# deepsound-project/pggan-pytorch

Hardware: AMD Instinct MI355X
Metric: images/sec, PGGAN full train step (D+GP step + G step + Adam) at 1024x1024 (higher is better)
Workload: dtype f32; 1 GPU; BASELINE config 5: PGGAN 1024x1024 net (fmap_base 4096, C=3, latent 512), stage depth 8 = 1024x1024, alpha 1.00, minibatch 3/GPU (reference schedule), Trainer.train(): WGAN-GP + Adam(0,0.99) at lr 0, fp32; resolution=1024, depth=8, minibatch_per_gpu=3, global_batch=3, parallelism=dp1, fmap_base=4096, hip_graphs=False

## Files before the change

### include/pggan_hip_debug.h

```cpp
#ifndef PGGAN_HIP_DEBUG_H
#define PGGAN_HIP_DEBUG_H

#ifdef __cplusplus
extern "C" {
#endif

const char* pg_debug_last_conv_kernel(void);
const char* pg_debug_last_wino_kernel(void);
const char* pg_debug_last_wino_wgrad_kernel(void);

enum pg_tune_key {
    PG_TUNE_CONV_TILE = 0,
    PG_TUNE_WGRAD = 1,
    PG_TUNE_SPLITK = 2,
    PG_TUNE_PATH = 3
};
enum pg_wgrad_cfg {
    PG_WGRAD_32x16_128PX = 1,
    PG_WGRAD_64x16_64PX = 3,
    PG_WGRAD_TILE_NOT_STRIP = 20
};
enum pg_path {
    PG_PATH_NO_THIN = 2,
    PG_PATH_NO_SMALLMAP_SPLIT = 8,
    PG_PATH_SMALLMAP_SPLIT_2304 = 9,
    PG_PATH_UNFUSED_PIXELNORM = 11,
    PG_PATH_NO_THIN_POOL16 = 17,
    PG_PATH_TILE_NOT_STRIP = 20,
    PG_PATH_K4_ONE_WORKGROUP = 21
};
int pg_debug_set_tuning(int key, int value);
int pg_debug_set_wino(int vec);
int pg_debug_set_wino_ksplit(int n);
int pg_debug_set_wino_epi(int mode);

#ifdef __cplusplus
}
#endif
#endif
```

### pggan-pytorch_amd/csrc/conv_api.hip

```cpp
#include "convp.h"

__thread char pgk::g_last_kernel[96] = "";
__thread int pgk::g_tune[4] = {-1, -1, -1, -1};

namespace {

using namespace pgk;

__device__ __forceinline__ void pack_dgrad_tile(const float* __restrict__ w, float* __restrict__ wt, int KS, int Cout, int Cin,
                                                int tap, int ci_b, int co_b)
{
    __shared__ float tile[32][33];
    const int kh = tap / KS, kw = tap % KS;
    const int otap = (KS - 1 - kh) * KS + (KS - 1 - kw);
    const int tx = threadIdx.x & 31, ty = threadIdx.x >> 5;
    for (int r = ty; r < 32; r += 8) {
        const int co = co_b + r, ci = ci_b + tx;
        tile[r][tx] = (co < Cout && ci < Cin) ? w[((size_t)tap * Cout + co) * Cin + ci] : 0.f;
    }
    __syncthreads();
    for (int r = ty; r < 32; r += 8) {
        const int ci = ci_b + r, co = co_b + tx;
        if (ci < Cin && co < Cout) wt[((size_t)otap * Cin + ci) * Cout + co] = tile[tx][r];
    }
// ... 32 lines not shown
    if (want.ypool && !pooled)
        return pg_avgpool2_fwd(want.y, want.pool_other, want.ypool, want.N, want.Hout >> 1, want.Wout >> 1, want.Cout, want.pool_a, want.pool_b, stream);
    if (want.yup) return pg_avgpool2_bwd(want.y, want.upmask, want.yup, want.N, want.Hout, want.Wout, want.Cout, want.up_mul, want.mask_slope, stream);
    if (want.pn_r) return pg_pixelnorm_fwd(want.y, want.y, want.pn_r, P, want.Cout, want.pn_eps, stream);
    if (want.pnb_y) return pg_pixelnorm_lrelu_bwd(want.y, want.pnb_y, want.pnb_r, want.y, P, want.Cout, want.mask_slope, stream);
    return 0;
}

static bool thin_shape(const ConvP& p, bool channels)
{
    return channels && p.KS == 3 && p.pad == 1 && (p.Wout & 31) == 0 && (p.Hout & 7) == 0 && g_tune[PG_TUNE_PATH] != PG_PATH_NO_THIN;
}

static ConvP conv_request(const float* x, const float* w, const float* bias, const float* mask, float* y,
                          int N, int Hin, int Win, int Cin, int Cout, int KS, int pad, float scale, float slope, float mask_slope)
{
    ConvP p;
    p.x = x; p.w = w; p.bias = bias; p.mask = mask; p.y = y;
    p.N = N; p.Hin = Hin; p.Win = Win; p.Cin = Cin; p.Cout = Cout; p.KS = KS; p.pad = pad;
    p.scale = scale; p.slope = slope; p.mask_slope = mask_slope;
    return p;
}

static int conv2d_impl(ConvP& p, int flags, pg_stream_t stream)
{
    if (!p.x || !p.w || !p.y || p.N <= 0 || p.Hin <= 0 || p.Win <= 0 || p.Cin <= 0 || p.Cout <= 0) return PG_E_ARG;
    if ((p.Cin & 3) || (p.Cout & 3)) return PG_E_ALIGN;
    const int KS = p.KS, Cin = p.Cin, Cout = p.Cout;
    p.ups = flags & PG_FLAG_UPSAMPLE;
    p.mask_bytes = (flags & PG_FLAG_MASK_BYTES) ? 1 : 0; p.y_bytes = (flags & PG_FLAG_Y_BYTES) ? 1 : 0;
    if (flags & PG_FLAG_SIGNS_OUT) {
        if (!p.mask || p.mask_bytes) return PG_E_ARG;
        p.ysigns = reinterpret_cast<unsigned char*>(const_cast<float*>(p.mask));
        p.mask = nullptr;
    }
    p.Hout = p.Hin + 2 * p.pad - KS + 1; p.Wout = p.Win + 2 * p.pad - KS + 1;
    if (p.Hout <= 0 || p.Wout <= 0 || !is_pow2(p.Hout) || !is_pow2(p.Wout)) return PG_E_UNSUP;
    if (p.ups && ((p.Hin | p.Win) & 1)) return PG_E_ARG;
    if (p.ypool && ((p.Hout | p.Wout) & 1)) return PG_E_ARG;
    if ((long long)p.N * p.Hin * p.Win * Cin >= (1ll << 31) || (long long)p.N * p.Hout * p.Wout * Cout >= (1ll << 31) ||
        (long long)KS * KS * Cout * Cin >= (1ll << 31)) return PG_E_UNSUP;
    const ConvP want = p;
    if (KS != 3) p.ypool = nullptr;
    p.yup = nullptr; p.pn_r = nullptr; p.pnb_y = nullptr;
    hipStream_t s = (hipStream_t)stream;
    int rc;
    if (p.mask_bytes || p.y_bytes || p.ysigns) {
        if (KS != 3 || (p.y_bytes && !p.ypool) || want.pn_r || want.pnb_y) return PG_E_UNSUP;
        p.yup = want.yup;
        const bool thin_plain = !p.y_bytes && !p.yup && !p.ypool && ((Cout == 8 && (Cin == 8 || Cin == 16)) || (Cout == 16 && Cin == 8 && p.mask));
        const bool thin_pool = g_tune[PG_TUNE_PATH] != PG_PATH_NO_THIN_POOL16 && !p.yup && p.ypool && Cout == 16 && Cin == 8;
        return thin_shape(p, thin_plain || thin_pool) ? dispatch_thin(p, s) : dispatch_conv_tile(p, s);
    }
    const bool thin_pn = thin_shape(p, Cout == 8 && (Cin == 8 || Cin == 16));
    if (want.pnb_y && want.pnb_r && KS == 3 && Cout <= 32) {
        p.pnb_y = want.pnb_y;
        rc = thin_pn ? dispatch_thin(p, s) : dispatch_conv_tile(p, s);
        if (rc != PG_E_UNSUP) return rc;
        p.pnb_y = nullptr;
    }
    if (want.pn_r && KS == 3 && Cout <= 32 && !p.mask && g_tune[PG_TUNE_PATH] != PG_PATH_UNFUSED_PIXELNORM) {
        p.pn_r = want.pn_r;
        rc = thin_pn ? dispatch_thin(p, s) : dispatch_conv_tile(p, s);
        if (rc != PG_E_UNSUP) return rc;
// ... 10 lines not shown
    else if (k4_layer(p, KS))
        rc = launch_k4_conv(p, s);
    else
        rc = dispatch_conv_tile(p, s);
    if (rc) return rc;
    return second_pass(want, p.ypool && p.ksplit == 1, stream);
}

extern "C" int pg_conv2d_nhwc(const float* x, const float* w, const float* bias, const float* mask, float* y,
                              int N, int Hin, int Win, int Cin, int Cout, int KS, int pad, int ups,
                              float scale, float slope, float mask_slope, pg_stream_t stream)
{
    ConvP p = conv_request(x, w, bias, mask, y, N, Hin, Win, Cin, Cout, KS, pad, scale, slope, mask_slope);
    return conv2d_impl(p, ups, stream);
}

extern "C" int pg_conv2d_pixelnorm_nhwc(const float* x, const float* w, const float* bias, float* y, float* r,
                                        int N, int Hin, int Win, int Cin, int Cout, int KS, int pad, int ups,
                                        float scale, float slope, float eps, pg_stream_t stream)
{
    if (!r) return PG_E_ARG;
    ConvP p = conv_request(x, w, bias, nullptr, y, N, Hin, Win, Cin, Cout, KS, pad, scale, slope, 0.2f);
    p.pn_r = r; p.pn_eps = eps;
    return conv2d_impl(p, ups, stream);
}

extern "C" int pg_conv2d_pnbwd_nhwc(const float* x, const float* w, const float* ysaved, const float* r, float* y,
                                    int N, int Hin, int Win, int Cin, int Cout, int KS, int pad,
                                    float scale, float slope, pg_stream_t stream)
{
    if (!ysaved) return PG_E_ARG;
    ConvP p = conv_request(x, w, nullptr, nullptr, y, N, Hin, Win, Cin, Cout, KS, pad, scale, 1.0f, slope);
    p.pnb_y = ysaved; p.pnb_r = r;
    return conv2d_impl(p, 0, stream);
}

extern "C" int pg_conv2d_unpool_nhwc(const float* x, const float* w, const float* upmask, float* y, float* yup,
                                     int N, int Hin, int Win, int Cin, int Cout, int KS, int pad, int flags,
                                     float scale, float up_mul, float mask_slope, pg_stream_t stream)
{
    if (!yup) return PG_E_ARG;
    ConvP p = conv_request(x, w, nullptr, nullptr, y, N, Hin, Win, Cin, Cout, KS, pad, scale, 1.0f, mask_slope);
    p.yup = yup; p.upmask = upmask; p.up_mul = up_mul;
    return conv2d_impl(p, flags & PG_FLAG_MASK_BYTES, stream);
}

extern "C" int pg_conv2d_pool_nhwc(const float* x, const float* w, const float* bias, const float* mask, float* y,
// ... 93 lines not shown
```

### pggan-pytorch_amd/csrc/conv_strip.hip

```cpp
#include "convp.h"

#ifndef PG_STRIP_ABL
#define PG_STRIP_ABL 0
#endif

namespace {

using pgk::ConvP;
using pgk::pg_sign_byte;
using pgk::pg_sign_factors;
using pgk::g_last_kernel; using pgk::set_smem; using pgk::SMEM_ANY;

constexpr int SW = 64;
constexpr int RP = SW + 2;
constexpr int RB = 4;
constexpr int NBLK = 3;

enum { EPI_GENERIC = 0, EPI_FWD = 1, EPI_MASK = 2, EPI_PN = 3, EPI_PNB = 4 };

struct SArgs {
    const float* x; const float* w; const float* bias; const void* mask; float* y;
    unsigned char* ysigns; float* pn_r; const float* pnb_y; const float* pnb_r; float* ypool; const float* pool_other;
    float scale, slope, mask_slope, pn_eps, pool_a, pool_b;
    int H, W, ups, mask_bytes, y_bytes, pool_only;
    int strips, segs, seg_rows;
    const unsigned char* gbytes; float gmul, gslope;
    const float* rgb_w; const float* rgb_b; float rgb_scale, rgb_slope; int rgbC; unsigned char* xsigns;
    float* t_out; const float* t_w; const float* t_b; float t_scale; int tC, t_sc, t_sco, t_only;
    const float* fw_img; float* fw_dw; float* fw_db; float fw_scale;
};

template <int CIN> struct Blk {
    static constexpr int C4 = CIN / 4;
    static constexpr int USED = C4 * RB * RP;
    static constexpr int NWI = (USED + 63) / 64;
    static constexpr int NI = (NWI + 3) / 4;
    static constexpr int SLOTS = NWI * 64;
};

typedef __attribute__((address_space(3))) const char* lds_cptr;
typedef __attribute__((address_space(3))) const f32x4* lds_v4ptr;

__device__ __forceinline__ pg_u32x4 rsrc_words(const void* base, unsigned bytes)
{
    const unsigned long long a = (unsigned long long)base;
    return pg_u32x4{(unsigned)__builtin_amdgcn_readfirstlane((int)(unsigned)a),
                    (unsigned)__builtin_amdgcn_readfirstlane((int)((unsigned)(a >> 32) & 0xffffu)), bytes, 0x00020000u};
}
__device__ __forceinline__ void buf_store4(__amdgpu_buffer_rsrc_t r, unsigned voff, float4 v)
{
    __builtin_amdgcn_raw_buffer_store_b128(pg_u32x4{__float_as_uint(v.x), __float_as_uint(v.y), __float_as_uint(v.z), __float_as_uint(v.w)},
                                           r, (int)voff, 0, 0);
}

constexpr int RGB_MAXC = 3;
template <int COUT, int CIN, int EPI, bool WREG, int GM, int XM = 0>
__device__ __forceinline__ void conv_strip_body(const SArgs& p)
{
    constexpr bool GATH = GM != 0;
    using B = Blk<CIN>;
    constexpr int C4 = B::C4;
    constexpr int QO = COUT / 4, QP = 16 / QO, PXG = 4 * QP;
    constexpr int GPR = 32 / PXG, G = 2 * GPR;
    constexpr int BLKB = B::SLOTS * 16;
    constexpr bool GEN = EPI == EPI_GENERIC;
    extern __shared__ __align__(16) float lds[];
    constexpr int WS = CIN == 16 ? CIN + 4 : CIN;
    float* wl = lds + NBLK * B::SLOTS * 4;
    const int tid = threadIdx.x, lane = tid & 63, wave = __builtin_amdgcn_readfirstlane(tid >> 6);
    const int blk = lane >> 2, j = lane & 3, qo = blk % QO, qp = blk / QO;

    int t = (int)pg_xcd_remap(blockIdx.x, gridDim.x);
    const int strip = __builtin_amdgcn_readfirstlane(t % p.strips); t /= p.strips;
    const int seg = __builtin_amdgcn_readfirstlane(t % p.segs), n = __builtin_amdgcn_readfirstlane(t / p.segs);
    const int r0 = seg * p.seg_rows, ow0 = strip * SW;
    const int niter = p.seg_rows / RB;
    const int xH = p.ups ? (p.H >> 1) : p.H, xW = p.ups ? (p.W >> 1) : p.W;
    const unsigned npix = (unsigned)(p.H * p.W);

    const unsigned rowbytes = 4u * (unsigned)(xW * CIN);
    unsigned voff[B::NI], vstep[B::NI];
    const unsigned blkstep = (p.ups ? 2u : 4u) * rowbytes;
#pragma unroll
    for (int i = 0; i < B::NI; ++i) {
        const int sl = (i * 4 + wave) * 64 + lane;
        const int q = sl / (RB * RP), rem = sl - q * (RB * RP);
        const int m = rem / RP, px = rem - m * RP;
        const int col = ow0 - 1 + px, row = r0 - 1 + m;
        const bool ok = sl < B::USED && (unsigned)col < (unsigned)p.W;
        voff[i] = ok ? (unsigned)(p.ups ? (row >> 1) : row) * rowbytes + 4u * (unsigned)((p.ups ? (col >> 1) : col) * CIN + 4 * q) : PG_OOB;
        vstep[i] = ok ? blkstep : 0u;
    }
    const size_t ximg = (size_t)xH * xW * CIN;
    const pg_u32x4 rxs = rsrc_words(p.x + (size_t)n * ximg, (unsigned)(ximg * 4));
    const unsigned lds0 = (unsigned)(size_t)(__attribute__((address_space(3))) char*)lds;
    const unsigned wdst = __builtin_amdgcn_readfirstlane(lds0 + (unsigned)wave * 1024u);
    auto dma16 = [&](unsigned vo, unsigned dst) {
        unsigned keep;
        asm volatile("s_mov_b32 %0, m0\n\ts_mov_b32 m0, %3\n\ts_nop 0\n\tbuffer_load_dwordx4 %1, %2, 0 offen lds\n\ts_mov_b32 m0, %0"
                     : "=&s"(keep) : "v"(vo), "s"(rxs), "s"(dst) : "memory");
    };
    auto issue_block = [&](int pos) {
#pragma unroll
        for (int i = 0; i < B::NI; ++i) {
            if (i * 4 + wave < B::NWI) dma16(voff[i], wdst + (unsigned)pos * BLKB + (unsigned)i * 4096u);
            voff[i] += vstep[i];
        }
    };

    constexpr int NG = GATH ? (B::USED + 255) / 256 : 1;
    unsigned cvo[NG], cvs[NG], bvo[NG], bvs[NG];
    float4 gxr[NG];
// ... 83 lines not shown
                rrow[i] += RB;
            }
            return;
        }
#pragma unroll
        for (int i = 0; i < NG; ++i) {
            const int sl = i * 256 + tid;
            if (sl < B::SLOTS) {
                const float4 f = pg_sign_factors((unsigned char)gbr[i], p.gslope);
                const float4 v = gxr[i];
                *reinterpret_cast<float4*>(lds + (pos * B::SLOTS + sl) * 4) =
                    make_float4(v.x * (f.x * p.gmul), v.y * (f.y * p.gmul), v.z * (f.z * p.gmul), v.w * (f.w * p.gmul));
            }
        }
    };

    float4 wreg[WREG ? 9 : 1][WREG ? C4 : 1];
    if constexpr (WREG) {
#pragma unroll
        for (int tp = 0; tp < 9; ++tp)
#pragma unroll
            for (int c4 = 0; c4 < C4; ++c4)
                wreg[tp][c4] = *reinterpret_cast<const float4*>(p.w + ((size_t)(tp * COUT + 4 * qo + j) * CIN + 4 * c4));
    } else {
        for (int e = tid; e < 9 * COUT * C4; e += 256)
            *reinterpret_cast<float4*>(wl + (e / C4) * WS + 4 * (e % C4)) = *reinterpret_cast<const float4*>(p.w + 4 * e);
    }
    const float* wrow = wl + (4 * qo + j) * WS;

    if constexpr (GATH) {
        gather_load(); gather_store(0);
        gather_load(); gather_store(1);
    } else {
        issue_block(0);
        issue_block(1);
    }

    const int rp = wave >> 1;
    const int col0 = (wave & 1) * 32;
    const lds_cptr lbase = (lds_cptr)lds + (col0 + 4 * qp + j) * 16;

    const bool has_mask = (GEN && p.mask) || EPI == EPI_MASK;
    const bool mask_bytes = has_mask && p.mask_bytes;
    const bool has_pnb = (GEN && p.pnb_y) || EPI == EPI_PNB;
    const bool has_pn = (GEN && p.pn_r) || EPI == EPI_PN;
    const bool has_signs = (GEN || EPI == EPI_FWD) && p.ysigns;
    const bool has_pool = GEN && p.ypool;
    const bool y_bytes = GEN && p.y_bytes;
    const bool has_trgb = (XM & 1) != 0 && (EPI == EPI_PN || EPI == EPI_MASK) && p.t_out != nullptr;
    const bool has_fw = (XM & 2) != 0 && EPI == EPI_MASK && COUT == 8 && p.fw_dw != nullptr;
    const bool y_store = !(has_pool && p.pool_only) && !y_bytes && !((has_trgb || has_fw) && p.t_only);
    const __amdgpu_buffer_rsrc_t ry = y_bytes ? pg_make_rsrc((const unsigned char*)p.y + (size_t)n * npix * (COUT / 4), npix * (COUT / 4))
                                              : pg_make_rsrc(p.y + (size_t)n * npix * COUT, npix * COUT * 4u);
    __amdgpu_buffer_rsrc_t rmask = ry, rsig = ry, rpnr = ry, rpnby = ry, rpnbr = ry;
    if (has_mask) rmask = mask_bytes ? pg_make_rsrc((const unsigned char*)p.mask + (size_t)n * npix * (COUT / 4), npix * (COUT / 4))
                                     : pg_make_rsrc((const float*)p.mask + (size_t)n * npix * COUT, npix * COUT * 4u);
    if (has_signs) rsig = pg_make_rsrc(p.ysigns + (size_t)n * npix * (COUT / 4), npix * (COUT / 4));
    if (has_pn) rpnr = pg_make_rsrc(p.pn_r + (size_t)n * npix, npix * 4u);
    if (has_pnb) {
        rpnby = pg_make_rsrc(p.pnb_y + (size_t)n * npix * COUT, npix * COUT * 4u);
        rpnbr = pg_make_rsrc(p.pnb_r + (size_t)n * npix, npix * 4u);
    }
    const unsigned pix0 = (unsigned)((r0 + 2 * rp) * p.W + ow0 + col0 + 4 * qp + j);
    float4 bv = make_float4(0.f, 0.f, 0.f, 0.f);
    if (!has_mask && p.bias) bv = *reinterpret_cast<const float4*>(p.bias + 4 * qo);
    float tw[RGB_MAXC][4], tb[RGB_MAXC];
    float aw[4][RGB_MAXC], ab[4], fi[G][RGB_MAXC];
#pragma unroll
    for (int k = 0; k < 4; ++k) {
        ab[k] = 0.f;
#pragma unroll
        for (int c = 0; c < RGB_MAXC; ++c) aw[k][c] = 0.f;
    }
    __amdgpu_buffer_rsrc_t rfimg = ry;
    if (has_fw) rfimg = pg_make_rsrc(p.fw_img + (size_t)n * npix * p.tC, npix * (unsigned)p.tC * 4u);
    __amdgpu_buffer_rsrc_t rtout = ry;
    if (has_trgb) {
        rtout = pg_make_rsrc(p.t_out + (size_t)n * npix * p.tC, npix * (unsigned)p.tC * 4u);
#pragma unroll
        for (int c = 0; c < RGB_MAXC; ++c) {
#pragma unroll
            for (int k = 0; k < 4; ++k) tw[c][k] = c < p.tC ? p.t_w[c * p.t_sc + (4 * qo + k) * p.t_sco] : 0.f;
            tb[c] = (c < p.tC && p.t_b) ? p.t_b[c] : 0.f;
        }
    }

    f32x4 acc[G], acc2[G];
    auto compute = [&](auto ph_, auto rp_) {
        constexpr int PH = decltype(ph_)::value, RPAIR = decltype(rp_)::value;
#pragma unroll
        for (int g = 0; g < G; ++g) { acc[g] = f32x4{0.f, 0.f, 0.f, 0.f}; acc2[g] = f32x4{0.f, 0.f, 0.f, 0.f}; }
#pragma unroll
        for (int tp = 0; tp < ((PG_STRIP_ABL & 4) ? 1 : 9); ++tp) {
            const int dy = tp / 3, dx = tp % 3;
#pragma unroll
            for (int c4 = 0; c4 < C4; ++c4) {
                float4 a;
                if constexpr (WREG) a = wreg[tp][c4];
                else a = *reinterpret_cast<const float4*>(wrow + tp * COUT * WS + 4 * c4);
                f32x4 bq[G];
#pragma unroll
                for (int g = 0; g < G; ++g) {
                    const int m = 2 * RPAIR + g / GPR + dy;
                    const int pos = m < RB ? PH : (PH + 1) % NBLK;
                    const int off = ((pos * B::SLOTS) + c4 * (RB * RP) + (m & (RB - 1)) * RP + (g % GPR) * PXG + dx) * 16;
                    bq[g] = *(lds_v4ptr)(lbase + off);
                }
#pragma unroll
                for (int g = 0; g < G; ++g) acc[g] = __builtin_amdgcn_mfma_f32_4x4x1f32(a.x, bq[g][0], acc[g], 0, 0, 0);
#pragma unroll
                for (int g = 0; g < G; ++g) acc2[g] = __builtin_amdgcn_mfma_f32_4x4x1f32(a.y, bq[g][1], acc2[g], 0, 0, 0);
#pragma unroll
                for (int g = 0; g < G; ++g) acc[g] = __builtin_amdgcn_mfma_f32_4x4x1f32(a.z, bq[g][2], acc[g], 0, 0, 0);
#pragma unroll
// ... 104 lines not shown
                                       (ov[g].z + ov[g + GPR].z) * 0.25f, (ov[g].w + ov[g + GPR].w) * 0.25f);
                if (j & 1) continue;
                const unsigned pg_ = pix + (unsigned)(g * PXG);
                const unsigned oy = pg_ / (unsigned)p.W, ox = pg_ - oy * (unsigned)p.W;
                const size_t poff = (((size_t)n * (p.H >> 1) + (oy >> 1)) * (p.W >> 1) + (ox >> 1)) * COUT + 4 * qo;
                if (p.pool_other) {
                    const float4 q = *reinterpret_cast<const float4*>(p.pool_other + poff);
                    v.x = fmaf(v.x, p.pool_a, p.pool_b * q.x); v.y = fmaf(v.y, p.pool_a, p.pool_b * q.y);
                    v.z = fmaf(v.z, p.pool_a, p.pool_b * q.z); v.w = fmaf(v.w, p.pool_a, p.pool_b * q.w);
                } else if (p.pool_a != 1.f) { v.x *= p.pool_a; v.y *= p.pool_a; v.z *= p.pool_a; v.w *= p.pool_a; }
                *reinterpret_cast<float4*>(p.ypool + poff) = v;
            }
        }
    };

    int nstores = (y_bytes || y_store) ? G : 0;
    if (has_signs) nstores += G;
    if (has_pn) nstores += G;
    if (has_pool) nstores += GPR;
    if (has_trgb) nstores += G * p.tC;
    if (PG_STRIP_ABL & 2) nstores = 0;
    nstores = __builtin_amdgcn_readfirstlane(nstores);
    auto wait_dma = [&]() {
        if constexpr (EPI == EPI_MASK || EPI == EPI_PNB || EPI == EPI_PN) {
            static_assert(G == 2, "");
            if (!has_trgb && !has_fw) {
                if constexpr (EPI == EPI_PN) asm volatile("s_waitcnt vmcnt(4)" ::: "memory");
                else asm volatile("s_waitcnt vmcnt(2)" ::: "memory");
            } else switch (nstores) {
                case 2: asm volatile("s_waitcnt vmcnt(2)" ::: "memory"); break;
                case 4: asm volatile("s_waitcnt vmcnt(4)" ::: "memory"); break;
                case 6: asm volatile("s_waitcnt vmcnt(6)" ::: "memory"); break;
                case 8: asm volatile("s_waitcnt vmcnt(8)" ::: "memory"); break;
                case 10: asm volatile("s_waitcnt vmcnt(10)" ::: "memory"); break;
                default: asm volatile("s_waitcnt vmcnt(0)" ::: "memory"); break;
            }
        }
        else switch (nstores) {
            case 0: asm volatile("s_waitcnt vmcnt(0)" ::: "memory"); break;
            case 1: asm volatile("s_waitcnt vmcnt(1)" ::: "memory"); break;
            case 2: asm volatile("s_waitcnt vmcnt(2)" ::: "memory"); break;
            case 3: asm volatile("s_waitcnt vmcnt(3)" ::: "memory"); break;
            case 4: asm volatile("s_waitcnt vmcnt(4)" ::: "memory"); break;
            case 5: asm volatile("s_waitcnt vmcnt(5)" ::: "memory"); break;
            default: asm volatile("s_waitcnt vmcnt(6)" ::: "memory"); break;
        }
    };
    unsigned pix = pix0;
    const unsigned pixstep = (unsigned)(RB * p.W);
    auto step = [&](int it, auto ph_) {
        constexpr int PH = decltype(ph_)::value;
        if constexpr (!GATH) {
            if (it == 0 || (PG_STRIP_ABL & 2)) asm volatile("s_waitcnt vmcnt(0)" ::: "memory");
            else wait_dma();
        }
        __syncthreads();
        const bool more = it + 2 <= niter;
        if constexpr (GATH) { if (more) gather_load(); }
        else if (more && !((PG_STRIP_ABL & 1) && it > 0)) issue_block((PH + 2) % NBLK);
        prefetch_epilogue(pix);
        __builtin_amdgcn_sched_barrier(0);
        if (rp == 0) compute(ph_, std::integral_constant<int, 0>{});
        else compute(ph_, std::integral_constant<int, 1>{});
        if constexpr (GATH) { if (more) gather_store((PH + 2) % NBLK); }
        epilogue(pix);
        pix += pixstep;
    };
    for (int it = 0; it < niter; it += 3) {
        step(it, std::integral_constant<int, 0>{});
        if (it + 1 < niter) step(it + 1, std::integral_constant<int, 1>{});
        if (it + 2 < niter) step(it + 2, std::integral_constant<int, 2>{});
    }
// ... 25 lines not shown
        };
        float a = 0.f;
        if (tid < 32) a = (lds[(0 * 2 + q2) * 16 + i] + lds[(1 * 2 + q2) * 16 + i]) + (lds[(2 * 2 + q2) * 16 + i] + lds[(3 * 2 + q2) * 16 + i]);
        if (tid < 32) commit(a);
    }
}

template <int COUT, int CIN, int EPI, bool WREG, bool GATH>
__global__ __launch_bounds__(256, GATH ? 2 : (WREG ? 3 : 4)) void conv_strip_kernel(SArgs p)
{
    conv_strip_body<COUT, CIN, EPI, WREG, GATH ? 1 : 0>(p);
}

template <int EPI, bool WREG, int XM>
__global__ __launch_bounds__(256, 3) void conv_strip_x_kernel(SArgs p)
{
    conv_strip_body<8, 8, EPI, WREG, 0, XM>(p);
}

template <int EPI>
__global__ __launch_bounds__(256, 2) void conv_strip_rgb_kernel(SArgs p)
{
    conv_strip_body<8, 8, EPI, false, 2>(p);
}

template <int COUT, int CIN, int EPI, bool WREG, bool GATH = false>
int launch_strip(const SArgs& a, int N, hipStream_t s)
{
    using B = Blk<CIN>;
    const size_t smem = (size_t)NBLK * B::SLOTS * 16 + (WREG ? 0 : (size_t)9 * COUT * (CIN == 16 ? CIN + 4 : CIN) * 4);
    auto kern = conv_strip_kernel<COUT, CIN, EPI, WREG, GATH>;
    if (int rc = set_smem(kern, smem, SMEM_ANY)) return rc;
    snprintf(g_last_kernel, sizeof(g_last_kernel), "conv_strip_kernel<%d, %d, %d, %s, %s>", COUT, CIN, EPI, WREG ? "true" : "false", GATH ? "true" : "false");
    hipLaunchKernelGGL(kern, dim3((unsigned)(N * a.strips * a.segs)), dim3(256), smem, s, a);
    return (int)hipGetLastError();
}

template <int EPI, bool WREG, int XM>
int launch_strip_x(const SArgs& a, int N, hipStream_t s)
{
    const size_t smem = (size_t)NBLK * Blk<8>::SLOTS * 16 + (WREG ? 0 : (size_t)9 * 8 * 8 * 4);
    auto kern = conv_strip_x_kernel<EPI, WREG, XM>;
    if (int rc = set_smem(kern, smem, SMEM_ANY)) return rc;
    snprintf(g_last_kernel, sizeof(g_last_kernel), "conv_strip_x_kernel<%d, %s, %d>", EPI, WREG ? "true" : "false", XM);
    hipLaunchKernelGGL(kern, dim3((unsigned)(N * a.strips * a.segs)), dim3(256), smem, s, a);
    return (int)hipGetLastError();
// ... 219 lines not shown
    return (seg < 16 || (seg % RB) || (H % seg)) ? 0 : seg;
}

constexpr bool STRIP_WREG = true;

}

int pgk::launch_conv_strip(ConvP& p, hipStream_t s)
{
    if (p.KS != 3 || p.pad != 1 || p.yup || p.ksplit != 1) return PG_E_UNSUP;
    if ((p.Wout % SW) || (p.Hout % 16) || p.Hout != p.Hin || p.Wout != p.Win) return PG_E_UNSUP;
    if (!(p.Cout == 8 && (p.Cin == 8 || p.Cin == 16))) return PG_E_UNSUP;
    if ((long long)p.Hin * p.Win * 16 * 4 >= (1ll << 31)) return PG_E_UNSUP;
    const int seg = strip_seg_rows(p.N, p.Hout, p.Wout);
    if (!seg) return PG_E_UNSUP;
    SArgs a{};
    a.x = p.x; a.w = p.w; a.bias = p.bias; a.mask = p.mask; a.y = p.y;
    a.ysigns = p.ysigns; a.pn_r = p.pn_r; a.pnb_y = p.pnb_y; a.pnb_r = p.pnb_r; a.ypool = p.ypool; a.pool_other = p.pool_other;
    a.scale = p.scale; a.slope = p.slope; a.mask_slope = p.mask_slope; a.pn_eps = p.pn_eps; a.pool_a = p.pool_a; a.pool_b = p.pool_b;
    a.H = p.Hout; a.W = p.Wout; a.ups = p.ups; a.mask_bytes = p.mask_bytes; a.y_bytes = p.y_bytes; a.pool_only = p.pool_only;
    a.strips = p.Wout / SW; a.segs = p.Hout / seg; a.seg_rows = seg;
    a.gbytes = p.gbytes; a.gmul = p.gmul; a.gslope = p.gslope;
    if (p.gbytes) {
        if (!p.ups || p.bias || p.ypool || p.y_bytes || p.pnb_y || p.pn_r || p.ysigns) return PG_E_UNSUP;
        if (p.Cin == 8) return p.mask ? launch_strip<8, 8, EPI_MASK, false, true>(a, p.N, s)
                                      : launch_strip<8, 8, EPI_FWD, false, true>(a, p.N, s);
        return p.mask ? launch_strip<8, 16, EPI_MASK, false, true>(a, p.N, s)
                      : launch_strip<8, 16, EPI_FWD, false, true>(a, p.N, s);
    }
    int epi = EPI_GENERIC;
    if (!p.ypool && !p.y_bytes) {
        if (p.pnb_y && !p.mask && !p.pn_r && !p.ysigns) epi = EPI_PNB;
        else if (p.pn_r && !p.mask && !p.pnb_y && !p.ysigns) epi = EPI_PN;
        else if (p.mask && !p.pnb_y && !p.pn_r) epi = EPI_MASK;
        else if (!p.mask && !p.pnb_y && !p.pn_r) epi = EPI_FWD;
    }
    if (p.Cin == 8) return launch_strip_epi<8, 8, STRIP_WREG>(a, epi, p.N, s);
    return launch_strip_epi<8, 16, false>(a, epi, p.N, s);
}

int pgk::launch_conv_strip_fromrgb(const float* img, const float* rgb_w, const float* rgb_b, float rgb_scale, float rgb_slope,
                                   unsigned char* x_signs, const float* w, const float* bias, float* y, unsigned char* y_signs,
                                   int N, int C, int H, int W, int Cmid, int Cout, float scale, float slope,
                                   hipStream_t s)
{
    if (C > RGB_MAXC || Cmid != 8 || Cout != 8 || (W % SW) || (H % 16)) return PG_E_UNSUP;
    if ((long long)H * W * 16 * 4 >= (1ll << 31)) return PG_E_UNSUP;
    const int seg = strip_seg_rows(N, H, W);
    if (!seg) return PG_E_UNSUP;
    SArgs a{};
    a.x = img; a.w = w; a.bias = bias; a.y = y; a.ysigns = y_signs;
    a.scale = scale; a.slope = slope; a.mask_slope = 1.f; a.pool_a = 1.f;
    a.H = H; a.W = W; a.strips = W / SW; a.segs = H / seg; a.seg_rows = seg;
    a.rgb_w = rgb_w; a.rgb_b = rgb_b; a.rgb_scale = rgb_scale; a.rgb_slope = rgb_slope; a.rgbC = C; a.xsigns = x_signs;
    const size_t smem = (size_t)NBLK * Blk<8>::SLOTS * 16 + (size_t)9 * 8 * 8 * 4;
    auto kern = conv_strip_rgb_kernel<EPI_FWD>;
    if (int rc = set_smem(kern, smem, SMEM_ANY)) return rc;
    snprintf(g_last_kernel, sizeof(g_last_kernel), "conv_strip_rgb_kernel<%d>", (int)EPI_FWD);
    hipLaunchKernelGGL(kern, dim3((unsigned)(N * a.strips * a.segs)), dim3(256), smem, s, a);
// ... 65 lines not shown
```

### pggan-pytorch_amd/engine.py

```python
import collections as _collections
import contextlib as _contextlib
import os
import weakref as _weakref

import torch

from . import ops
from . import saved


def _check_dev(t, what):
    if not torch.is_tensor(t) or not t.is_cuda:
        raise RuntimeError('%s must be a tensor on the MI355X device (no CPU path exists); got %s'
                           % (what, getattr(t, 'device', type(t))))
    if t.dtype != torch.float32:
        raise RuntimeError('%s must be float32' % what)
    return t.contiguous()


USE_WINOGRAD = True
WINO_MIN_WORKGROUPS = 32
_WINO_MIN_CHANNELS = 8
_WINO_MIN_COUT = 16
_WINO_WGRAD_MIN_CHANNELS = 16
FALLBACKS = _collections.Counter()
USE_SIGN_BYTES = True
SIGN_BYTES_MIN_H = 64
USE_LAZY_UNPOOL = True


def _live_conv_layers(net):
    depth = int(net.depth)
    if not hasattr(net, 'linear'):
        return [lay for _, lay in net.stage_convs(depth)]
    blocks = list(net.blocks)[len(net.blocks) - 1 - depth:]
    return [m for b in blocks for m in (b.c1, b.c2)]


def _derived(net):
    net._ensure_buffers()
    rt = net._rt
    key = (net._param_version, int(net.depth))
    if rt.derived_ver == key:
        return
# ... 373 lines not shown
                         layer.c, ups=ups)


def _flush_wgrad(layer):
    pend = layer._pending_wgrad
    if pend is None:
        return
    layer._pending_wgrad = None
    x, gz, N, Hin = pend
    with _on_side(x, gz):
        ops.conv2d_wgrad_wino(x, gz, layer._gw, None, N, Hin, Hin, layer.c)


_ONES = {}


def _ones(n, device):
    key = (n, str(device))
    if key not in _ONES:
        _ONES[key] = torch.ones(n, device=device, dtype=torch.float32)
    return _ONES[key]


def generator_forward(G, z, save=False, out=None, pair_out=None):
    wait_pending(G)
    ops.require_gpu()
    G._sync_version()
    z = _check_dev(z, 'latents')
    N, L = z.shape
    if L != G.latent_size or L % 4:
        raise ValueError('latent size %d (expected %d, multiple of 4)' % (L, G.latent_size))
    depth, alpha = int(G.depth), float(G.alpha)
    C = G.num_channels
    b0 = G.block0
    G._ensure_buffers()
    ctx = saved.GContext(N=N, depth=depth, alpha=alpha, recs=[])
    if G.normalize_latents:
        zn, _ = ops.pixelnorm_fwd(z, G.eps)
    else:
        zn = z
    ctx.zn = zn

    def layer(x, lay, H, ups=False):
        if lay.pixelnorm:
            u = _wino(lay, N, H, lay.conv.weight.shape[2]) if lay.ksize == 3 else None
            if u is not None and u.shape[1] <= 32:
                return ops.conv2d_wino_pixelnorm(x, u, lay.conv.bias.data, N, H, H, lay.c, lay.slope, lay.eps, ups=ups)
            if u is not None:
                y = ops.conv2d_wino(x, u, lay.conv.bias.data, N, H, H, lay.c, lay.slope, ups=ups)
                return ops.pixelnorm_fwd(y, lay.eps, inplace=True)
            return ops.conv2d_pixelnorm(x, lay.conv.weight.data, lay.conv.bias.data, N, H, H, lay.ksize, lay.pad, lay.c,
                                        lay.slope, lay.eps, ups=ups)
        return _conv(x, lay, N, H, ups=ups), None

    y1, r1 = layer(zn.view(N, 1, 1, L), b0.c1, 1)
    y2, r2 = layer(y1, b0.c2, 4)
    ctx.y1, ctx.r1, ctx.y2, ctx.r2 = y1, r1, y2, r2
    def to_rgb(h, t, H, out_mul=1.0, prev=None, prev_mul=0.0):
        if pair_out is None:
            return ops.torgb_fwd(h, t.conv.weight.data, t.conv.bias.data, N, C, H, H, t.c, out_mul=out_mul, prev=prev, prev_mul=prev_mul, out=out)
        n2 = N // 2
        return tuple(ops.torgb_fwd(h[a:b], t.conv.weight.data, t.conv.bias.data, n2, C, H, H, t.c, out_mul=out_mul,
                                   prev=prev[a:b] if prev is not None else None, prev_mul=prev_mul, out=o)
                     for (a, b), o in zip(((0, n2), (n2, N)), pair_out))
    if depth == 0:
        img = to_rgb(y2, b0.toRGB, 4)
        return (img, ctx) if save else img
    h, H = y2, 4
    for i in range(depth):
        blk = G.blocks[i]
        H *= 2
        a1, ra1 = layer(h, blk.c1, H, ups=True)
        img = None
# ... 639 lines not shown
EARLY_G_FORWARD = True
EARLY_G_MIN_RES = 256
EARLY_G_MODE = 'auto'
_EARLY_G_BATCHED_MAX_RES = 4


def early_g_mode(depth):
    if not EARLY_G_FORWARD:
        return None
    res = 4 * 2 ** int(depth)
    if EARLY_G_MODE == 'auto':
        return 'batched' if res <= _EARLY_G_BATCHED_MAX_RES else 'side' if res >= EARLY_G_MIN_RES else None
    return EARLY_G_MODE if (res >= EARLY_G_MIN_RES or res <= _EARLY_G_BATCHED_MAX_RES) else None
EARLY_G_STATS = {'passes': 0, 'used': 0, 'dropped': 0}


class EarlyG(object):
    __slots__ = ('fake', 'ctx', 'latents', 'stamp', 'event')


def d_step_generator(D, G, latents, out):
    req = D._rt.early_g_request if early_g_mode(G.depth) == 'batched' else None
    if req is None or req[0] is not G or tuple(req[1].shape) != tuple(latents.shape):
        return generator_forward(G, latents, out=out)
    D._rt.early_g_request = None
    zg = _check_dev(req[1], 'latents')
    N = latents.shape[0]
    z2 = torch.empty((2 * N,) + tuple(latents.shape[1:]), device=latents.device, dtype=torch.float32)
    ops.axpby_mask(latents, a=1.0, out=z2[:N])
    ops.axpby_mask(zg, a=1.0, out=z2[N:])
    eg = EarlyG()
    eg.fake = torch.empty_like(out)
    (img, _), ctx = generator_forward(G, z2, save=True, pair_out=(out, eg.fake))
    eg.ctx = ctx.slice(N, 2 * N)
    eg.event = torch.cuda.Event()
    _record_event(eg.event, torch.cuda.current_stream(torch._C._cuda_getDevice()))
    eg.latents = zg
    eg.stamp = (G._param_version, int(G.depth), float(G.alpha))
    G._rt.early_fwd = eg
    EARLY_G_STATS['passes'] += 1
    return img


def request_early_g(D, G, latents):
    D._rt.early_g_request = (G, latents)


def _early_g_on_side(D, main, side):
    req = D._rt.take('early_g_request')
    if req is None or early_g_mode(req[0].depth) != 'side':
        return
    G, z = req
    z = _check_dev(z, 'latents')
    with torch.cuda.stream(side):
        probe('D.early_g_start')
        eg = EarlyG()
        eg.fake, eg.ctx = generator_forward(G, z, save=True)
        eg.event = torch.cuda.Event()
        _record_event(eg.event, side)
        probe('D.early_g_end')
    eg.fake.record_stream(main)
    for t in saved.tensors(eg.ctx):
        t.record_stream(main)
    eg.latents = z
    eg.stamp = (G._param_version, int(G.depth), float(G.alpha))
    G._rt.early_fwd = eg
    EARLY_G_STATS['passes'] += 1


def take_early_g(G, latents):
    eg = G._rt.take('early_fwd')
    if eg is None:
        return None
    if eg.latents is not latents or eg.stamp != (G._param_version, int(G.depth), float(G.alpha)):
        EARLY_G_STATS['dropped'] += 1
        return None
    _wait_event(torch.cuda.current_stream(torch._C._cuda_getDevice()), eg.event)
    EARLY_G_STATS['used'] += 1
    return eg

# ... 52 lines not shown
    if aug is None:
        ops.axpby_mask(real, a=1.0, out=x2[:N])
        d_step_generator(D, G, latents, x2[N:])
    else:
        _augmented(aug, real, table[:N], out=x2[:N])
        _augmented(aug, d_step_generator(D, G, latents, torch.empty_like(real)), table[N:], out=x2[N:])
    s, ctx = d_forward(D, x2, groups=2)
    d_cost, d_real_loss, d_fake_loss, gscore = _d_loss_block(objective, s, None, N)
    _count_real_signs(aug, s, N)
    return d_cost, d_real_loss, d_fake_loss, saved.DLossState(D=D, ctx=ctx, gscore=gscore, N=N, scores=s)


def g_loss_forward(G, D, latents, objective, table=None):
    ops.require_gpu()
    latents = _check_dev(latents, 'latents')
    table = _step_table(objective, table, latents.shape[0])
    D._sync_version()
    G._sync_version()
    probe('G.start')
    eg = take_early_g(G, latents)
    if eg is not None:
        fake, gctx = eg.fake, eg.ctx
    else:
        fake, gctx = generator_forward(G, latents, save=True)
    probe('G.g_fwd_end')
    if table is not None:
        fake = _augmented(objective.augment, fake, table)
    s, dctx = d_forward(D, fake, 1, keep_input=False)
    g_cost, gscore = _g_loss_block(objective, s)
    probe('G.d_fwd_end')
    return g_cost, saved.GLossState(G=G, D=D, gctx=gctx, dctx=dctx, gscore=gscore, table=table)


def g_loss_backward(state, scale=1.0):
    G, D = state.G, state.D

    def sweep():
        gimg, _ = d_backward(D, state.dctx, state.gscore, full=False, want_gimg=True)
        if state.table is not None:
            gimg = ops.augment_adjoint(gimg, state.table)
        probe('G.d_bwd_end')
        return generator_backward(G, state.gctx, gimg)
    state.active_g = _backward(G, scale, sweep, ('G.g_bwd_end', 'G.wgrad_end'))
```

### pggan-pytorch_amd/ops.py

```python
import os as _os

import ctypes

import torch

from . import _lib

_C = _lib.CONSTANTS


def _stream():
    return torch._C._cuda_getCurrentRawStream(torch._C._cuda_getDevice())


WORKSPACE_BYTES = int(_os.environ.get('PGGAN_WORKSPACE_MB', '32')) << 20
_workspaces = {}
_capture_workspace = {}
_no_workspace_streams = set()


def workspace_bytes(kind, N, H, W, cin, cout):
    n = ctypes.c_size_t(0)
    _lib.call('pg_workspace_bytes', kind, N, H, W, cin, cout, ctypes.addressof(n))
    return int(n.value)
# ... 213 lines not shown


def conv2d_pool(x, w, bias, N, Hin, Win, ks, pad, scale, slope=1.0, mask=None, mask_slope=0.2, other=None, a=1.0, b=0.0,
                pool_only=False, y_bytes=False):
    cout, cin = w.shape[2], w.shape[3]
    ho, wo = Hin + 2 * pad - ks + 1, Win + 2 * pad - ks + 1
    flags = (FLAG_MASK_BYTES if _is_bytes(mask) else 0) | (FLAG_Y_BYTES if y_bytes else 0)
    if y_bytes:
        y = _empty((N, ho, wo, cout // 4), device=x.device, dtype=torch.uint8)
    else:
        y = _empty((N, ho, wo, cout), device=x.device, dtype=torch.float32)
    yp = _empty((N, ho // 2, wo // 2, cout), device=x.device, dtype=torch.float32)
    _lib.call('pg_conv2d_pool_nhwc', _p(x), _p(w), _p(bias), _p(mask), _p(y), _p(yp), _p(other), a, b, 1 if pool_only else 0,
              N, Hin, Win, cin, cout, ks, pad, flags, scale, slope, mask_slope, _stream())
    return y, yp


def conv2d_pixelnorm(x, w, bias, N, Hin, Win, ks, pad, scale, slope, eps=1e-8, ups=False):
    cout, cin = w.shape[2], w.shape[3]
    ho, wo = Hin + 2 * pad - ks + 1, Win + 2 * pad - ks + 1
    y = torch.empty((N, ho, wo, cout), device=x.device, dtype=torch.float32)
    r = torch.empty((N * ho * wo,), device=x.device, dtype=torch.float32)
    _lib.call('pg_conv2d_pixelnorm_nhwc', _p(x), _p(w), _p(bias), _p(y), _p(r), N, Hin, Win, cin, cout, ks, pad,
              1 if ups else 0, scale, slope, eps, _stream())
    return y, r


def conv2d_pixelnorm_torgb(x, w, bias, t_w, t_b, N, C, H, W, scale, slope, t_scale, eps=1e-8, out=None):
    cout, cin = w.shape[2], w.shape[3]
    y = torch.empty((N, H, W, cout), device=x.device, dtype=torch.float32)
    r = torch.empty((N * H * W,), device=x.device, dtype=torch.float32)
    if out is None:
        out = torch.empty((N, C, H, W), device=x.device, dtype=torch.float32)
    _lib.call('pg_conv2d_pixelnorm_torgb_nhwc', _p(x), _p(w), _p(bias), _p(y), _p(r), _p(t_w), _p(t_b), t_scale, _p(out),
              N, C, H, W, cin, cout, scale, slope, eps, _stream())
    return y, r, out


def conv2d_pnbwd(x, w, ysaved, r, N, Hin, Win, ks, pad, scale, slope):
    cout, cin = w.shape[2], w.shape[3]
    ho, wo = Hin + 2 * pad - ks + 1, Win + 2 * pad - ks + 1
    y = torch.empty((N, ho, wo, cout), device=x.device, dtype=torch.float32)
    _lib.call('pg_conv2d_pnbwd_nhwc', _p(x), _p(w), _p(ysaved), _p(r), _p(y), N, Hin, Win, cin, cout, ks, pad, scale, slope, _stream())
    return y


def conv2d_unpool(x, w, N, Hin, Win, ks, pad, scale, upmask=None, mul=1.0, mask_slope=0.2):
# ... 1300 lines not shown
```

Baseline: 299.2 images/sec.

## Collapse nearest-upsample into 2x2 subpixel kernels for 1024px generator conv

Adds a collapsed path for the upsample+3x3 conv+PixelNorm layer at 1024 resolution with 16->8 channels. Nearest upsample followed by a 3x3 conv is rewritten as four 2x2 phase-specific kernels applied to the low-resolution input, with pre-summed weights. This cuts MACs per output from 9 to 4 taps and halves input staging in LDS. The cost is a new MFMA inner loop, modified LDS/pixel indexing, and weight pre-summing per block, with a fallback to the old path if unsupported.

```diff
diff --git a/include/pggan_hip_debug.h b/include/pggan_hip_debug.h
--- a/include/pggan_hip_debug.h
+++ b/include/pggan_hip_debug.h
@@ -27,7 +27,8 @@
     PG_PATH_UNFUSED_PIXELNORM = 11,
     PG_PATH_NO_THIN_POOL16 = 17,
     PG_PATH_TILE_NOT_STRIP = 20,
-    PG_PATH_K4_ONE_WORKGROUP = 21
+    PG_PATH_K4_ONE_WORKGROUP = 21,
+    PG_PATH_NO_UPS_COLLAPSE = 22
 };
 int pg_debug_set_tuning(int key, int value);
 int pg_debug_set_wino(int vec);
diff --git a/pggan-pytorch_amd/csrc/conv_api.hip b/pggan-pytorch_amd/csrc/conv_api.hip
--- a/pggan-pytorch_amd/csrc/conv_api.hip
+++ b/pggan-pytorch_amd/csrc/conv_api.hip
@@ -78,7 +78,7 @@
     return p;
 }
 
-static int conv2d_impl(ConvP& p, int flags, pg_stream_t stream)
+static int conv2d_impl(ConvP& p, int flags, pg_stream_t stream, bool collapse = false)
 {
     if (!p.x || !p.w || !p.y || p.N <= 0 || p.Hin <= 0 || p.Win <= 0 || p.Cin <= 0 || p.Cout <= 0) return PG_E_ARG;
     if ((p.Cin & 3) || (p.Cout & 3)) return PG_E_ALIGN;
@@ -96,6 +96,11 @@
     if (p.ypool && ((p.Hout | p.Wout) & 1)) return PG_E_ARG;
     if ((long long)p.N * p.Hin * p.Win * Cin >= (1ll << 31) || (long long)p.N * p.Hout * p.Wout * Cout >= (1ll << 31) ||
         (long long)KS * KS * Cout * Cin >= (1ll << 31)) return PG_E_UNSUP;
+    if (collapse && g_tune[PG_TUNE_PATH] != PG_PATH_NO_UPS_COLLAPSE) {
+        if (p.mask || p.mask_bytes || p.y_bytes || p.ysigns || p.ypool || p.yup || p.pnb_y) return PG_E_UNSUP;
+        p.ups = 2;
+        return launch_conv_strip(p, (hipStream_t)stream);
+    }
     const ConvP want = p;
     if (KS != 3) p.ypool = nullptr;
     p.yup = nullptr; p.pn_r = nullptr; p.pnb_y = nullptr;
@@ -152,7 +157,8 @@
     if (!r) return PG_E_ARG;
     ConvP p = conv_request(x, w, bias, nullptr, y, N, Hin, Win, Cin, Cout, KS, pad, scale, slope, 0.2f);
     p.pn_r = r; p.pn_eps = eps;
-    return conv2d_impl(p, ups, stream);
+    if (ups < 0 || ups > 2) return PG_E_ARG;
+    return conv2d_impl(p, ups ? PG_FLAG_UPSAMPLE : 0, stream, ups == 2);
 }
 
 extern "C" int pg_conv2d_pnbwd_nhwc(const float* x, const float* w, const float* ysaved, const float* r, float* y,
diff --git a/pggan-pytorch_amd/csrc/conv_strip.hip b/pggan-pytorch_amd/csrc/conv_strip.hip
--- a/pggan-pytorch_amd/csrc/conv_strip.hip
+++ b/pggan-pytorch_amd/csrc/conv_strip.hip
@@ -30,9 +30,11 @@
     const float* fw_img; float* fw_dw; float* fw_db; float fw_scale;
 };
 
-template <int CIN> struct Blk {
+constexpr int RPC = SW / 2 + 2;
+template <int CIN, bool UPC = false> struct Blk {
     static constexpr int C4 = CIN / 4;
-    static constexpr int USED = C4 * RB * RP;
+    static constexpr int RPX = UPC ? RPC : RP;
+    static constexpr int USED = C4 * RB * RPX;
     static constexpr int NWI = (USED + 63) / 64;
     static constexpr int NI = (NWI + 3) / 4;
     static constexpr int SLOTS = NWI * 64;
@@ -54,14 +56,17 @@
 }
 
 constexpr int RGB_MAXC = 3;
-template <int COUT, int CIN, int EPI, bool WREG, int GM, int XM = 0>
+template <int COUT, int CIN, int EPI, bool WREG, int GM, int XM = 0, bool UPC = false>
 __device__ __forceinline__ void conv_strip_body(const SArgs& p)
 {
     constexpr bool GATH = GM != 0;
-    using B = Blk<CIN>;
+    static_assert(!UPC || (COUT == 8 && !WREG && GM == 0 && XM == 0 && EPI == EPI_PN), "collapsed form: 8 couts, PixelNorm epilogue");
+    using B = Blk<CIN, UPC>;
     constexpr int C4 = B::C4;
+    constexpr int RPX = B::RPX;
     constexpr int QO = COUT / 4, QP = 16 / QO, PXG = 4 * QP;
-    constexpr int GPR = 32 / PXG, G = 2 * GPR;
+    constexpr int GPR = 32 / PXG, G = UPC ? 4 : 2 * GPR;
+    constexpr int SROWS = UPC ? 2 * RB : RB;
     constexpr int BLKB = B::SLOTS * 16;
     constexpr bool GEN = EPI == EPI_GENERIC;
     extern __shared__ __align__(16) float lds[];
@@ -74,20 +79,22 @@
     const int strip = __builtin_amdgcn_readfirstlane(t % p.strips); t /= p.strips;
     const int seg = __builtin_amdgcn_readfirstlane(t % p.segs), n = __builtin_amdgcn_readfirstlane(t / p.segs);
     const int r0 = seg * p.seg_rows, ow0 = strip * SW;
-    const int niter = p.seg_rows / RB;
+    const int niter = p.seg_rows / SROWS;
     const int xH = p.ups ? (p.H >> 1) : p.H, xW = p.ups ? (p.W >> 1) : p.W;
     const unsigned npix = (unsigned)(p.H * p.W);
 
     const unsigned rowbytes = 4u * (unsigned)(xW * CIN);
     unsigned voff[B::NI], vstep[B::NI];
-    const unsigned blkstep = (p.ups ? 2u : 4u) * rowbytes;
+    const unsigned blkstep = ((p.ups && !UPC) ? 2u : 4u) * rowbytes;
 #pragma unroll
     for (int i = 0; i < B::NI; ++i) {
         const int sl = (i * 4 + wave) * 64 + lane;
-        const int q = sl / (RB * RP), rem = sl - q * (RB * RP);
-        const int m = rem / RP, px = rem - m * RP;
-        const int col = ow0 - 1 + px, row = r0 - 1 + m;
-        const bool ok = sl < B::USED && (unsigned)col < (unsigned)p.W;
+        const int q = sl / (RB * RPX), rem = sl - q * (RB * RPX);
+        const int m = rem / RPX, px = rem - m * RPX;
+        const int col = UPC ? (ow0 >> 1) - 1 + px : ow0 - 1 + px, row = UPC ? (r0 >> 1) - 1 + m : r0 - 1 + m;
+        const bool ok = sl < B::USED && (unsigned)col < (unsigned)(UPC ? xW : p.W);
+        if constexpr (UPC) voff[i] = ok ? (unsigned)row * rowbytes + 4u * (unsigned)(col * CIN + 4 * q) : PG_OOB;
+        else
         voff[i] = ok ? (unsigned)(p.ups ? (row >> 1) : row) * rowbytes + 4u * (unsigned)((p.ups ? (col >> 1) : col) * CIN + 4 * q) : PG_OOB;
         vstep[i] = ok ? blkstep : 0u;
     }
@@ -217,11 +224,23 @@
 #pragma unroll
             for (int c4 = 0; c4 < C4; ++c4)
                 wreg[tp][c4] = *reinterpret_cast<const float4*>(p.w + ((size_t)(tp * COUT + 4 * qo + j) * CIN + 4 * c4));
+    } else if constexpr (UPC) {
+        for (int e = tid; e < 16 * COUT * C4; e += 256) {
+            const int c4 = e % C4, co = (e / C4) % COUT, bb = (e / (C4 * COUT)) & 1, t = e / (2 * C4 * COUT);
+            const int a = t >> 2, dy = (t >> 1) & 1, dx = t & 1;
+            const int rlo = a == 0 ? dy : 2 * dy, rhi = a == 0 ? 2 * dy : 1 + dy;
+            const int clo = bb == 0 ? dx : 2 * dx, chi = bb == 0 ? 2 * dx : 1 + dx;
+            auto tap = [&](int r, int c) { return *reinterpret_cast<const float4*>(p.w + ((size_t)((r * 3 + c) * COUT + co) * CIN + 4 * c4)); };
+            auto add4 = [](float4 u, float4 v) { return make_float4(__fadd_rn(u.x, v.x), __fadd_rn(u.y, v.y), __fadd_rn(u.z, v.z), __fadd_rn(u.w, v.w)); };
+            auto rowsum = [&](int r) { return clo == chi ? tap(r, clo) : add4(tap(r, clo), tap(r, chi)); };
+            const float4 k = rlo == rhi ? rowsum(rlo) : add4(rowsum(rlo), rowsum(rhi));
+            *reinterpret_cast<float4*>(wl + ((t * 2 + bb) * COUT + co) * WS + 4 * c4) = k;
+        }
     } else {
         for (int e = tid; e < 9 * COUT * C4; e += 256)
             *reinterpret_cast<float4*>(wl + (e / C4) * WS + 4 * (e % C4)) = *reinterpret_cast<const float4*>(p.w + 4 * e);
     }
-    const float* wrow = wl + (4 * qo + j) * WS;
+    const float* wrow = wl + ((UPC ? (qp & 1) * COUT : 0) + 4 * qo + j) * WS;
 
     if constexpr (GATH) {
         gather_load(); gather_store(0);
@@ -233,7 +252,7 @@
 
     const int rp = wave >> 1;
     const int col0 = (wave & 1) * 32;
-    const lds_cptr lbase = (lds_cptr)lds + (col0 + 4 * qp + j) * 16;
+    const lds_cptr lbase = (lds_cptr)lds + (UPC ? (col0 >> 1) + 4 * (qp >> 1) + j + (qp & 1) : col0 + 4 * qp + j) * 16;
 
     const bool has_mask = (GEN && p.mask) || EPI == EPI_MASK;
     const bool mask_bytes = has_mask && p.mask_bytes;
@@ -256,7 +275,8 @@
         rpnby = pg_make_rsrc(p.pnb_y + (size_t)n * npix * COUT, npix * COUT * 4u);
         rpnbr = pg_make_rsrc(p.pnb_r + (size_t)n * npix, npix * 4u);
     }
-    const unsigned pix0 = (unsigned)((r0 + 2 * rp) * p.W + ow0 + col0 + 4 * qp + j);
+    const unsigned pix0 = UPC ? (unsigned)((r0 + 4 * rp) * p.W + ow0 + col0 + 2 * (4 * (qp >> 1) + j) + (qp & 1))
+                              : (unsigned)((r0 + 2 * rp) * p.W + ow0 + col0 + 4 * qp + j);
     float4 bv = make_float4(0.f, 0.f, 0.f, 0.f);
     if (!has_mask && p.bias) bv = *reinterpret_cast<const float4*>(p.bias + 4 * qo);
     float tw[RGB_MAXC][4], tb[RGB_MAXC];
@@ -285,6 +305,36 @@
         constexpr int PH = decltype(ph_)::value, RPAIR = decltype(rp_)::value;
 #pragma unroll
         for (int g = 0; g < G; ++g) { acc[g] = f32x4{0.f, 0.f, 0.f, 0.f}; acc2[g] = f32x4{0.f, 0.f, 0.f, 0.f}; }
+        if constexpr (UPC) {
+#pragma unroll
+            for (int c4 = 0; c4 < C4; ++c4) {
+                f32x4 px[4][2], wk[8];
+#pragma unroll
+                for (int r = 0; r < 4; ++r)
+#pragma unroll
+                    for (int dx = 0; dx < 2; ++dx) {
+                        const int m = 2 * RPAIR + r;
+                        const int pos = m < RB ? PH : (PH + 1) % NBLK;
+                        px[r][dx] = *(lds_v4ptr)(lbase + ((pos * B::SLOTS) + c4 * (RB * RPX) + (m & (RB - 1)) * RPX + dx) * 16);
+                    }
+#pragma unroll
+                for (int t = 0; t < 8; ++t) {
+                    const float4 a = *reinterpret_cast<const float4*>(wrow + t * 2 * COUT * WS + 4 * c4);
+                    wk[t] = f32x4{a.x, a.y, a.z, a.w};
+                }
+#pragma unroll
+                for (int k = 0; k < 4; ++k)
+#pragma unroll
+                    for (int tp = 0; tp < 4; ++tp)
+#pragma unroll
+                        for (int g = 0; g < G; ++g) {
+                            const int il = g >> 1, a = g & 1, dy = tp >> 1, dx = tp & 1;
+                            f32x4& d = (k & 1) ? acc2[g] : acc[g];
+                            d = __builtin_amdgcn_mfma_f32_4x4x1f32(wk[a * 4 + tp][k], px[il + a + dy][dx][k], d, 0, 0, 0);
+                        }
+                __builtin_amdgcn_sched_barrier(0);
+            }
+        } else
 #pragma unroll
         for (int tp = 0; tp < ((PG_STRIP_ABL & 4) ? 1 : 9); ++tp) {
             const int dy = tp / 3, dx = tp % 3;
@@ -435,7 +485,11 @@
     if (PG_STRIP_ABL & 2) nstores = 0;
     nstores = __builtin_amdgcn_readfirstlane(nstores);
     auto wait_dma = [&]() {
-        if constexpr (EPI == EPI_MASK || EPI == EPI_PNB || EPI == EPI_PN) {
+        if constexpr (UPC) {
+            if (nstores == 8) asm volatile("s_waitcnt vmcnt(8)" ::: "memory");
+            else asm volatile("s_waitcnt vmcnt(0)" ::: "memory");
+        }
+        else if constexpr (EPI == EPI_MASK || EPI == EPI_PNB || EPI == EPI_PN) {
             static_assert(G == 2, "");
             if (!has_trgb && !has_fw) {
                 if constexpr (EPI == EPI_PN) asm volatile("s_waitcnt vmcnt(4)" ::: "memory");
@@ -460,7 +514,7 @@
         }
     };
     unsigned pix = pix0;
-    const unsigned pixstep = (unsigned)(RB * p.W);
+    const unsigned pixstep = (unsigned)(SROWS * p.W);
     auto step = [&](int it, auto ph_) {
         constexpr int PH = decltype(ph_)::value;
         if constexpr (!GATH) {
@@ -532,6 +586,24 @@
 __global__ __launch_bounds__(256, 2) void conv_strip_rgb_kernel(SArgs p)
 {
     conv_strip_body<8, 8, EPI, false, 2>(p);
+}
+
+template <int EPI>
+__global__ __launch_bounds__(256, 3) void conv_strip_upc_kernel(SArgs p)
+{
+    conv_strip_body<8, 16, EPI, false, 0, 0, true>(p);
+}
+
+template <int EPI>
+int launch_strip_upc(const SArgs& a, int N, hipStream_t s)
+{
+    using B = Blk<16, true>;
+    const size_t smem = (size_t)NBLK * B::SLOTS * 16 + (size_t)16 * 8 * (16 + 4) * 4;
+    auto kern = conv_strip_upc_kernel<EPI>;
+    if (int rc = set_smem(kern, smem, SMEM_ANY)) return rc;
+    snprintf(g_last_kernel, sizeof(g_last_kernel), "conv_strip_upc_kernel<%d>", EPI);
+    hipLaunchKernelGGL(kern, dim3((unsigned)(N * a.strips * a.segs)), dim3(256), smem, s, a);
+    return (int)hipGetLastError();
 }
 
 template <int COUT, int CIN, int EPI, bool WREG, bool GATH = false>
@@ -797,7 +869,7 @@
     a.strips = p.Wout / SW; a.segs = p.Hout / seg; a.seg_rows = seg;
     a.gbytes = p.gbytes; a.gmul = p.gmul; a.gslope = p.gslope;
     if (p.gbytes) {
-        if (!p.ups || p.bias || p.ypool || p.y_bytes || p.pnb_y || p.pn_r || p.ysigns) return PG_E_UNSUP;
+        if (p.ups != 1 || p.bias || p.ypool || p.y_bytes || p.pnb_y || p.pn_r || p.ysigns) return PG_E_UNSUP;
         if (p.Cin == 8) return p.mask ? launch_strip<8, 8, EPI_MASK, false, true>(a, p.N, s)
                                       : launch_strip<8, 8, EPI_FWD, false, true>(a, p.N, s);
         return p.mask ? launch_strip<8, 16, EPI_MASK, false, true>(a, p.N, s)
@@ -810,6 +882,8 @@
         else if (p.mask && !p.pnb_y && !p.pn_r) epi = EPI_MASK;
         else if (!p.mask && !p.pnb_y && !p.pn_r) epi = EPI_FWD;
     }
+    if (p.ups == 2)
+        return (p.Cin == 16 && epi == EPI_PN && (seg % (2 * RB)) == 0) ? launch_strip_upc<EPI_PN>(a, p.N, s) : PG_E_UNSUP;
     if (p.Cin == 8) return launch_strip_epi<8, 8, STRIP_WREG>(a, epi, p.N, s);
     return launch_strip_epi<8, 16, false>(a, epi, p.N, s);
 }
diff --git a/pggan-pytorch_amd/engine.py b/pggan-pytorch_amd/engine.py
--- a/pggan-pytorch_amd/engine.py
+++ b/pggan-pytorch_amd/engine.py
@@ -20,6 +20,7 @@
 
 USE_WINOGRAD = True
 WINO_MIN_WORKGROUPS = 32
+UPS_COLLAPSE_MIN_H = 1024
 _WINO_MIN_CHANNELS = 8
 _WINO_MIN_COUT = 16
 _WINO_WGRAD_MIN_CHANNELS = 16
@@ -439,7 +440,7 @@
     return _ONES[key]
 
 
-def generator_forward(G, z, save=False, out=None, pair_out=None):
+def generator_forward(G, z, save=False, out=None, pair_out=None, collapse=False):
     wait_pending(G)
     ops.require_gpu()
     G._sync_version()
@@ -466,6 +467,12 @@
             if u is not None:
                 y = ops.conv2d_wino(x, u, lay.conv.bias.data, N, H, H, lay.c, lay.slope, ups=ups)
                 return ops.pixelnorm_fwd(y, lay.eps, inplace=True)
+            if ups and collapse and H >= UPS_COLLAPSE_MIN_H and tuple(lay.conv.weight.shape[2:]) == (8, 16) and lay.ksize == 3:
+                try:
+                    return ops.conv2d_pixelnorm(x, lay.conv.weight.data, lay.conv.bias.data, N, H, H, lay.ksize, lay.pad, lay.c,
+                                                lay.slope, lay.eps, ups=2)
+                except ops.Unsupported:
+                    FALLBACKS['collapsed upsample %dx%d' % (H, H)] += 1
             return ops.conv2d_pixelnorm(x, lay.conv.weight.data, lay.conv.bias.data, N, H, H, lay.ksize, lay.pad, lay.c,
                                         lay.slope, lay.eps, ups=ups)
         return _conv(x, lay, N, H, ups=ups), None
@@ -1151,7 +1158,7 @@
 def d_step_generator(D, G, latents, out):
     req = D._rt.early_g_request if early_g_mode(G.depth) == 'batched' else None
     if req is None or req[0] is not G or tuple(req[1].shape) != tuple(latents.shape):
-        return generator_forward(G, latents, out=out)
+        return generator_forward(G, latents, out=out, collapse=True)
     D._rt.early_g_request = None
     zg = _check_dev(req[1], 'latents')
     N = latents.shape[0]
@@ -1160,7 +1167,7 @@
     ops.axpby_mask(zg, a=1.0, out=z2[N:])
     eg = EarlyG()
     eg.fake = torch.empty_like(out)
-    (img, _), ctx = generator_forward(G, z2, save=True, pair_out=(out, eg.fake))
+    (img, _), ctx = generator_forward(G, z2, save=True, pair_out=(out, eg.fake), collapse=True)
     eg.ctx = ctx.slice(N, 2 * N)
     eg.event = torch.cuda.Event()
     _record_event(eg.event, torch.cuda.current_stream(torch._C._cuda_getDevice()))
@@ -1184,7 +1191,7 @@
     with torch.cuda.stream(side):
         probe('D.early_g_start')
         eg = EarlyG()
-        eg.fake, eg.ctx = generator_forward(G, z, save=True)
+        eg.fake, eg.ctx = generator_forward(G, z, save=True, collapse=True)
         eg.event = torch.cuda.Event()
         _record_event(eg.event, side)
         probe('D.early_g_end')
@@ -1283,7 +1290,7 @@
     if eg is not None:
         fake, gctx = eg.fake, eg.ctx
     else:
-        fake, gctx = generator_forward(G, latents, save=True)
+        fake, gctx = generator_forward(G, latents, save=True, collapse=True)
     probe('G.g_fwd_end')
     if table is not None:
         fake = _augmented(objective.augment, fake, table)
diff --git a/pggan-pytorch_amd/ops.py b/pggan-pytorch_amd/ops.py
--- a/pggan-pytorch_amd/ops.py
+++ b/pggan-pytorch_amd/ops.py
@@ -259,7 +259,7 @@
     y = torch.empty((N, ho, wo, cout), device=x.device, dtype=torch.float32)
     r = torch.empty((N * ho * wo,), device=x.device, dtype=torch.float32)
     _lib.call('pg_conv2d_pixelnorm_nhwc', _p(x), _p(w), _p(bias), _p(y), _p(r), N, Hin, Win, cin, cout, ks, pad,
-              1 if ups else 0, scale, slope, eps, _stream())
+              2 if ups == 2 else (1 if ups else 0), scale, slope, eps, _stream())
     return y, r
 
 
```

Result: no change. 300.9 images/sec, median of 6 (+0.6%).
